# ostafen/smart

Measured on AMD Instinct MI355X. Metric: GB/s text scanned per GPU (bit-exact occ count), m=32 on 1 GiB rand128, higher is better.
Workload: dtype u8; 1 GPU; HOR m=32, 1.00 GiB rand128 per GPU; algorithm=hor, m=32, sigma=128, text_bytes_per_gpu=1073741824, patterns=2668, corpus=counter-based splitmix64 rand-sigma, seed 0x5EED0001, generated on device, ranks=1

## Files before the change

### smart_amd/csrc/api.cpp

```cpp
#include "../../include/smartgpu.h"

#include <hip/hip_runtime.h>
#include <rccl/rccl.h>

#include <dlfcn.h>

#include <algorithm>
#include <atomic>
#include <chrono>
#include <condition_variable>
#include <functional>
#include <mutex>
#include <thread>
#include <cstdarg>
#include <cstdio>
#include <cstring>
#include <string>
#include <vector>

#include "kernels.hpp"
#include "multi.hpp"
#include "multi_find.hpp"
#include "multi_find_host.hpp"
#include "pedit.hpp"
// ... 62 lines not shown
DeviceCtx* device_ctx(int device)
{
    int n = 0;
    if (hipGetDeviceCount(&n) != hipSuccess || n <= 0) {
        set_error("no HIP device available (hipGetDeviceCount)");
        return nullptr;
    }
    if (device < 0 || device >= n || device >= kMaxDevices) {
        set_error("device %d out of range (have %d)", device, n);
        return nullptr;
    }
    DeviceCtx& d = g_dev[device];
    HIP_TRY(hipSetDevice(device), return nullptr);
    if (!d.ready) {
        hipDeviceProp_t prop;
        HIP_TRY(hipGetDeviceProperties(&prop, device), return nullptr);
        d.num_cus = prop.multiProcessorCount;
        d.device = device;
        HIP_TRY(hipStreamCreateWithFlags(&d.stream, hipStreamNonBlocking), return nullptr);
        d.pinned_bytes = sg::kStagingBytes;
        HIP_TRY(hipHostMalloc(reinterpret_cast<void**>(&d.pinned), d.pinned_bytes, hipHostMallocDefault),
                return nullptr);
        HIP_TRY(hipHostMalloc(reinterpret_cast<void**>(&d.pinned_count), 64, hipHostMallocDefault),
                return nullptr);
        d.ready = true;
    }
    return &d;
}

DeviceCtx* device_ctx_ready(int device)
{
    if (device >= 0 && device < kMaxDevices && g_dev[device].ready) return &g_dev[device];
    return device_ctx(device);
}

constexpr unsigned long long kPoisonedCount = 1ull << 62;
bool count_poisoned(unsigned long long c)
{
    if (c < kPoisonedCount) return false;
    set_error("a scan kernel found its LDS segment displaced (static LDS in a kernel that addresses LDS by offset): count poisoned");
    return true;
}

double now_ms()
{
    using clk = std::chrono::steady_clock;
    return std::chrono::duration<double, std::milli>(clk::now().time_since_epoch()).count();
}

int probe_read_ms(const DeviceCtx* d, const uint8_t* first, uint64_t bytes, unsigned long long* sink, int reps, double* ms_per_pass)
{
    hipEvent_t e0 = nullptr, e1 = nullptr;
    const auto timed = [&]() -> int {
        HIP_TRY(hipEventCreate(&e0), return SMARTGPU_ERR_HIP);
        HIP_TRY(hipEventCreate(&e1), return SMARTGPU_ERR_HIP);
        sg::launch_probe_read(first, bytes, sink, d->num_cus, d->stream);
        hipEventRecord(e0, d->stream);
        for (int i = 0; i < reps; ++i) sg::launch_probe_read(first, bytes, sink, d->num_cus, d->stream);
        hipEventRecord(e1, d->stream);
        HIP_TRY(hipEventSynchronize(e1), return SMARTGPU_ERR_HIP);
        float ms = 0.f;
        hipEventElapsedTime(&ms, e0, e1);
        *ms_per_pass = ms / reps;
        return SMARTGPU_OK;
    };
    const int rc = timed();
    if (e0) hipEventDestroy(e0);
    if (e1) hipEventDestroy(e1);
    return rc;
}

}

struct smartgpu_text {
    int device = 0;
    uint64_t n = 0;
    uint8_t* base = nullptr;
    const uint8_t* data() const { return base + sg::kFrontPad; }
    uint32_t alphabet[8] = {0, 0, 0, 0, 0, 0, 0, 0};
    uint32_t four_shift = 7, four_symtab = 0, one_bit = 0xFF;
    sg::TextCodes codes() const { sg::TextCodes c; c.shift = four_shift; c.symtab = four_symtab; c.one = one_bit; return c; }
    double rate = -1.0;
    uint32_t* sample = nullptr;
};

struct smartgpu_plan {
    int device = 0;
    int algo = 0;
    uint32_t m = 0;
    sg::PlanWords words;
    uint8_t* blob = nullptr;
    uint8_t tail[sg::kTailRow] = {};
    uint8_t head[sg::kSampleRow] = {};
    unsigned long long* results = nullptr;
    unsigned long long* ext_results = nullptr;
    int ext_slots = 0;
    unsigned long long* slot_ptr(int slot) const { return ext_results ? ext_results + slot : results + slot; }
    int num_slots() const { return ext_results ? ext_slots : sg::kResultSlots; }
    hipEvent_t ev0[sg::kResultSlots] = {};
    hipEvent_t ev1[sg::kResultSlots] = {};
    bool timed[sg::kResultSlots] = {};
    double pre_ms = 0.0;
};

namespace {

smartgpu_text* text_alloc(uint64_t n, int device, DeviceCtx** ctx_out)
{
    DeviceCtx* d = device_ctx(device);
    if (!d) return nullptr;
    smartgpu_text* t = new smartgpu_text;
    t->device = device;
    t->n = n;
    const uint64_t total = sg::kFrontPad + n + sg::kBackPad;
    if (hipMalloc(reinterpret_cast<void**>(&t->base), total) != hipSuccess) {
        set_error("hipMalloc of %llu bytes failed", (unsigned long long)total);
        delete t;
        return nullptr;
    }
    if (hipMemsetAsync(t->base, 0, sg::kFrontPad, d->stream) != hipSuccess ||
        hipMemsetAsync(t->base + sg::kFrontPad + n, 0, sg::kBackPad, d->stream) != hipSuccess) {
        set_error("hipMemsetAsync of the text pads failed");
        hipFree(t->base);
        delete t;
        return nullptr;
    }
    *ctx_out = d;
    return t;
}

constexpr size_t kAlphabetScratchOff = 64;
static_assert(kAlphabetScratchOff + 32 <= sg::kFrontPad - (SMARTGPU_XSIZE + 256), "the scratch must lie below every byte a scan can read");
static_assert(sg::kHitSlotsOff >= kAlphabetScratchOff + 32 && sg::kHitSlotsOff + sg::kHitSlots * 128 <= sg::kFrontPad - (SMARTGPU_XSIZE + 256),
              "flush_hits' staging slots lie between the scratch and the bytes a scan can read");
bool text_alphabet(smartgpu_text* t, DeviceCtx* d)
{
    uint32_t* dev = reinterpret_cast<uint32_t*>(t->base + kAlphabetScratchOff);
    uint64_t hist[256] = {};
    unsigned long long* dev_hist = nullptr;
    const bool with_rate = sg::g_text_histogram && sg::rate_sample(t->n).bytes() >= 2;
    hipError_t e = hipMemsetAsync(dev, 0, 32, d->stream);
    if (e == hipSuccess && with_rate) e = hipMalloc(reinterpret_cast<void**>(&dev_hist), sizeof hist);
    if (e == hipSuccess && with_rate) e = hipMemsetAsync(dev_hist, 0, sizeof hist, d->stream);
    if (e == hipSuccess && t->n) e = sg::launch_text_alphabet(t->data(), t->n, dev, d->num_cus, d->stream);
    if (e == hipSuccess && with_rate) e = static_cast<hipError_t>(sg::g_text_histogram(t->data(), t->n, dev_hist, d->num_cus, d->stream));
    if (e == hipSuccess) e = hipMemcpyAsync(t->alphabet, dev, 32, hipMemcpyDeviceToHost, d->stream);
    if (e == hipSuccess && with_rate) e = hipMemcpyAsync(hist, dev_hist, sizeof hist, hipMemcpyDeviceToHost, d->stream);
    const hipError_t synced = hipStreamSynchronize(d->stream);
    if (e == hipSuccess) e = synced;
    if (dev_hist) (void)hipFree(dev_hist);
    if (e != hipSuccess) { set_error("text_alphabet failed: %s", hipGetErrorString(e)); return false; }
    t->rate = with_rate ? sg::text_repeat_rate(hist) : -1.0;
    if (!sg::four_symbol_codes(t->alphabet, &t->four_shift, &t->four_symtab)) t->four_shift = 7;
    t->one_bit = 0xFF;
    {
        uint32_t syms[3], ns = 0;
        for (uint32_t c = 0; c < 256 && ns < 3; ++c)
            if (t->alphabet[c >> 5] >> (c & 31) & 1u) syms[ns++] = c;
        if (ns == 1) syms[ns++] = syms[0];
        if (ns == 2) {
            uint32_t bit = 0;
            while (bit < 7 && ((syms[0] ^ syms[1]) >> bit & 1u) == 0) ++bit;
            const uint32_t s0 = (syms[0] >> bit & 1u) ? syms[1] : syms[0], s1 = (syms[0] >> bit & 1u) ? syms[0] : syms[1];
            t->one_bit = bit | (s0 << 8) | (s1 << 16);
        }
    }
    const uint32_t words[3] = {t->four_shift, t->four_symtab, t->one_bit};
    if (hipMemcpyAsync(t->base, words, 12, hipMemcpyHostToDevice, d->stream) != hipSuccess ||
        hipMemsetAsync(dev, 0, 32, d->stream) != hipSuccess ||
        hipStreamSynchronize(d->stream) != hipSuccess) {
        set_error("text_alphabet: writing the codes failed");
        return false;
    }
    return true;
}

bool text_no_alphabet(smartgpu_text* t, DeviceCtx* d)
{
    t->four_shift = 7;
    t->four_symtab = 0;
    t->one_bit = 0xFF;
    t->rate = -1.0;
    for (uint32_t& wv : t->alphabet) wv = 0xFFFFFFFFu;
    const uint32_t words[3] = {7u, 0u, 0xFFu};
    if (hipMemcpyAsync(t->base, words, 12, hipMemcpyHostToDevice, d->stream) != hipSuccess || hipStreamSynchronize(d->stream) != hipSuccess) {
        set_error("text upload: writing the codes failed");
        return false;
    }
    return true;
}

std::atomic<long long> g_text_sampling{64ll << 20};

void text_sample(smartgpu_text* t, DeviceCtx* d)
{
    const long long least = g_text_sampling.load(std::memory_order_relaxed);
    if (least < 0 || t->n < static_cast<uint64_t>(least) || !sg::g_sample_build) return;
    uint32_t* s = nullptr;
    if (hipMalloc(reinterpret_cast<void**>(&s), sg::sample_alloc_dwords(t->n) * 4) != hipSuccess) {
        (void)hipGetLastError();
        return;
    }
    if (sg::g_sample_build(t->data(), t->n, s, d->num_cus, d->stream) != hipSuccess || hipStreamSynchronize(d->stream) != hipSuccess) {
        (void)hipGetLastError();
        (void)hipFree(s);
        return;
    }
    t->sample = s;
}

int check_pattern(int algo, const uint8_t* P, uint32_t m, bool length_first = false)
{
    if (algo < 0 || algo >= SMARTGPU_NUM_ALGOS) { set_error("unknown algorithm id %d", algo); return SMARTGPU_ERR_ARG; }
    const bool na = m < sg::min_pattern(algo);
    if ((!na || length_first) && (!P || m < 1 || m > SMARTGPU_XSIZE)) { set_error("pattern length %u outside [1,%d]", m, SMARTGPU_XSIZE); return SMARTGPU_ERR_ARG; }
    if (na) { set_error("%s: not applicable for m < %u", sg::kAlgoNames[algo], sg::min_pattern(algo)); return SMARTGPU_NA; }
    return SMARTGPU_OK;
}

int check_search_args(int algo, const uint8_t* P, uint32_t m, const smartgpu_text* text,
                      uint64_t off, uint64_t n)
{
    const int rc = check_pattern(algo, P, m);
    if (rc != SMARTGPU_OK) return rc;
    if (!text) { set_error("text handle is NULL"); return SMARTGPU_ERR_ARG; }
    if (off > text->n || n > text->n - off) { set_error("range [%llu,+%llu) outside the text (%llu bytes)", (unsigned long long)off, (unsigned long long)n, (unsigned long long)text->n); return SMARTGPU_ERR_ARG; }
    return SMARTGPU_OK;
}

sg::ScanArgs make_args(const sg::PlanWords& pw, uint32_t m, const uint8_t* blob, unsigned long long* count, const smartgpu_text* text,
                       uint64_t off, uint64_t n)
{
    const uint64_t s_end = (n >= m) ? off + n - m + 1 : off;
    return sg::ScanArgs{text->data(), off, s_end, m, pw.halo,  0, pw.prefer_packed, pw.sparse, pw.so_off, blob, count};
}

struct QueuedScan { int algo; sg::ScanArgs a; sg::TextCodes codes; uint8_t tail[sg::kTailRow]; uint8_t head[sg::kSampleRow]; const uint32_t* sample; };
bool same_key(const sg::ScanArgs& x, const sg::ScanArgs& a) { return x.text == a.text && x.s_begin == a.s_begin && x.s_end == a.s_end && x.m == a.m && x.halo == a.halo; }
struct QueuedKey {
    sg::ScanArgs key;
    uint32_t n = 0;
    uint32_t streaming = 0;
    int64_t opened_ns = 0;
    bool fast = false;
    QueuedScan scans[sg::kLongMax];
    bool holds(const sg::ScanArgs& a) const { return same_key(key, a); }
    void take(const QueuedKey& o)
    {
        key = o.key;
        n = o.n;
        streaming = o.streaming;
        opened_ns = o.opened_ns;
        fast = o.fast;
        std::memcpy(static_cast<void*>(scans), static_cast<const void*>(o.scans), o.n * sizeof(QueuedScan));
    }
};
static_assert(std::is_trivially_copyable<QueuedScan>::value, "QueuedKey::take copies entries as bytes");
static_assert(SMARTGPU_XSIZE - 1 - sg::kGramCap + sg::kTailRow <= sg::kPatternBytes, "a long pass reads whole rows from a blob's pattern slot");
struct LaunchQueue {
    std::mutex mu;
    static constexpr uint32_t kKeys = 8;
    uint32_t nkeys = 0;
    QueuedKey keys[kKeys];
    void drop(uint32_t at) { for (--nkeys; at < nkeys; ++at) keys[at].take(keys[at + 1]); }
    uint32_t nfull = 0, full_next = 0;
    sg::ScanArgs full[kKeys];
    bool was_full(const sg::ScanArgs& a) const
    {
        for (uint32_t i = 0; i < nfull; ++i)
            if (same_key(full[i], a)) return true;
        return false;
    }
    void note_full(const sg::ScanArgs& a)
    {
        if (was_full(a)) return;
        if (nfull < kKeys) { full[nfull++] = a; return; }
        full[full_next] = a;
        full_next = (full_next + 1) % kKeys;
    }
    bool off = false;
    uint64_t launches = 0, passes = 0;
    uint64_t riders = 0;
    uint64_t sampled = 0;
};
LaunchQueue g_queue[kMaxDevices];
std::atomic<long long> g_coalesce_long{64ll << 20};
constexpr int kCoalesceNarrow = 8;
std::atomic<int> g_coalesce{sg::kPassMax};
std::atomic<int> g_coalesce_sample{1};
std::atomic<int> g_sample_grid{0};
bool pass_sampled(const uint32_t* sample, uint32_t m)
{
    return sample && m >= sg::kSampleMinM && sg::g_hor_sample && g_coalesce_sample.load(std::memory_order_relaxed) != 0;
}

int64_t host_ns()
{
    return std::chrono::duration_cast<std::chrono::nanoseconds>(std::chrono::steady_clock::now().time_since_epoch()).count();
}
constexpr int64_t kFastLeastNs = 10000;
int64_t pass_estimate_ns(uint64_t range, bool sampled)
{
    const uint64_t bytes = sampled ? range / (sg::kSampleStride / sg::kSampleGram) : range;
    return static_cast<int64_t>(bytes / 4400u);
}

hipError_t send_key(const DeviceCtx* d, LaunchQueue& q, QueuedKey& k)
{
    hipError_t e = k.n ? hipSetDevice(d->device) : hipSuccess;
    if (e != hipSuccess) {
        k.n = 0;
        k.streaming = 0;
        return e;
    }
    if (k.n == 1) {
        e = sg::launch_scan(k.scans[0].algo, k.scans[0].a, d->num_cus, d->stream, k.scans[0].codes);
    } else if (k.n > 1) {
        sg::MultiArgs ma;
        ma.text = k.key.text;
        ma.s_begin = k.key.s_begin;
        ma.s_end = k.key.s_end;
        ma.m = k.key.m;
        ma.halo = k.key.halo & 0xFFu;
        ma.np = k.n;
        const uint32_t* sample = k.scans[0].sample;
        if (pass_sampled(sample, k.key.m)) {
            const bool by_value = k.n <= sg::kSampleWidth;
            ma.stride = sg::kSampleRow;
            ma.width = by_value ? sg::kSampleWidth : sg::kSampleLongWidth;
            ma.reserved = by_value ? sg::kMultiByValue : sg::kMultiLong;
            for (uint32_t j = 0; j < k.n; ++j) {
                if (by_value) sg::sample_set(ma, j, k.scans[j].a.blob, k.scans[j].a.count, k.scans[j].head);
                else sg::multi_set_long(ma, j, k.scans[j].a.blob, k.scans[j].a.count);
            }
            e = sg::g_hor_sample(ma, sample, d->num_cus, g_sample_grid.load(std::memory_order_relaxed), d->stream);
            if (e == hipSuccess) ++q.sampled;
        } else {
            ma.stride = sg::tail_stride(k.key.m);
            if (k.n <= sg::pass_width(k.key.m)) {
                ma.width = sg::pass_width(k.key.m);
                ma.reserved = sg::kMultiByValue;
                for (uint32_t j = 0; j < k.n; ++j) sg::multi_set(ma, j, k.scans[j].a.blob, k.scans[j].a.count, k.scans[j].tail);
            } else {
                ma.width = sg::long_width(k.key.m);
                ma.reserved = sg::kMultiLong;
                for (uint32_t j = 0; j < k.n; ++j) sg::multi_set_long(ma, j, k.scans[j].a.blob, k.scans[j].a.count);
            }
            e = sg::g_hor_multi(ma, d->num_cus, d->stream);
        }
    }
    if (k.n && e == hipSuccess) ++q.passes;
    k.n = 0;
    k.streaming = 0;
    return e;
}

hipError_t flush_queue(const DeviceCtx* d)
{
    LaunchQueue& q = g_queue[d->device];
    std::lock_guard<std::mutex> lock(q.mu);
    hipError_t err = hipSuccess;
    for (uint32_t i = 0; i < q.nkeys; ++i) {
        const hipError_t e = send_key(d, q, q.keys[i]);
        if (e != hipSuccess && err == hipSuccess) err = e;
    }
    q.nkeys = 0;
    q.nfull = q.full_next = 0;
    return err;
}

void flush_all_queues()
{
    int current = -1;
    for (int i = 0; i < kMaxDevices; ++i) {
        if (!g_dev[i].ready) continue;
        {
            std::lock_guard<std::mutex> lock(g_queue[i].mu);
            if (g_queue[i].nkeys == 0) continue;
        }
        if (current < 0 && hipGetDevice(&current) != hipSuccess) return;
        if (hipSetDevice(i) == hipSuccess) (void)flush_queue(&g_dev[i]);
    }
    if (current >= 0) (void)hipSetDevice(current);
}

DeviceCtx* device_ctx_flushed(int device)
{
    DeviceCtx* d = device_ctx(device);
    if (!d) return nullptr;
    const hipError_t e = flush_queue(d);
    if (e != hipSuccess) { set_error("a queued launch failed: %s", hipGetErrorString(e)); return nullptr; }
    return d;
}

hipError_t queue_launch(const DeviceCtx* d, int algo, const sg::PlanWords& words, const sg::ScanArgs& a, const sg::TextCodes& codes,
                        double text_rate, const uint8_t (&tail)[sg::kTailRow], const uint8_t (&head)[sg::kSampleRow], const uint32_t* sample,
                        bool timed, bool* queued)
{
    *queued = false;
    if (a.s_end <= a.s_begin) return hipSuccess;
    const bool rider = !words.sparse;
    if (rider && (a.m < 8 || !sg::text_rate_streams(text_rate))) return hipSuccess;
    const sg::Route r = sg::route(algo, a.m, words, codes);
    if (r.to != sg::Launcher::hor || r.arg != 0) return hipSuccess;
    LaunchQueue& q = g_queue[d->device];
    std::lock_guard<std::mutex> lock(q.mu);
    if (!rider) ++q.launches;
    const int G = g_coalesce.load(std::memory_order_relaxed);
    if (timed || G < 2 || q.off || !sg::g_hor_multi) {
        if (!rider) ++q.passes;
        return hipSuccess;
    }
    hipError_t err = hipSuccess;
    uint32_t at = 0;
    while (at < q.nkeys && !q.keys[at].holds(a)) ++at;
    if (at == q.nkeys) {
        if (rider) return hipSuccess;
        if (q.nkeys == LaunchQueue::kKeys) {
            err = send_key(d, q, q.keys[0]);
            q.drop(0);
        }
        at = q.nkeys++;
        q.keys[at].key = a;
        q.keys[at].n = 0;
        q.keys[at].streaming = 0;
        q.keys[at].fast = false;
        q.keys[at].opened_ns = host_ns();
    }
    QueuedKey& k = q.keys[at];
    QueuedScan& qs = k.scans[k.n++];
    qs.algo = algo;
    qs.a = a;
    qs.codes = codes;
    std::memcpy(qs.tail, tail, sg::kTailRow);
    std::memcpy(qs.head, head, sg::kSampleRow);
    qs.sample = sample;
    if (rider) ++q.riders; else ++k.streaming;
    const bool sampled = pass_sampled(sample, a.m);
    const uint32_t room = sampled ? sg::kSampleWidth : sg::pass_width(a.m);
    const uint32_t long_room = sampled ? sg::kSampleLongWidth : sg::long_width(a.m);
    const uint32_t width = static_cast<uint32_t>(G) < room ? static_cast<uint32_t>(G) : room;
    const long long least = g_coalesce_long.load(std::memory_order_relaxed);
    const bool may_gather = G == sg::kPassMax && least >= 0 && a.s_end - a.s_begin >= static_cast<uint64_t>(least);
    const bool full = k.streaming >= width || k.n >= room;
    if (may_gather && full && !k.fast && k.n < long_room && !q.was_full(a)) {
        const int64_t waited = host_ns() - k.opened_ns;
        const int64_t pass_ns = pass_estimate_ns(a.s_end - a.s_begin, sampled);
        k.fast = pass_ns >= kFastLeastNs && waited >= 0 && waited / k.n * (long_room - k.n) < pass_ns;
    }
    const bool gather_on = may_gather && (k.fast || q.was_full(a));
    if (gather_on ? k.n >= long_room : full) {
        q.note_full(k.key);
        const hipError_t e = send_key(d, q, k);
        if (e != hipSuccess && err == hipSuccess) err = e;
        q.drop(at);
    }
    *queued = true;
    return err;
}

}

namespace sg {
hipError_t (*g_hor_multi)(const MultiArgs&, int, hipStream_t) = nullptr;
hipError_t (*g_hor_multi_find)(const MultiFindArgs&, int, hipStream_t) = nullptr;
hipError_t (*g_hor_sample)(const MultiArgs&, const uint32_t*, int, int, hipStream_t) = nullptr;
hipError_t (*g_sample_build)(const uint8_t*, uint64_t, uint32_t*, int, hipStream_t) = nullptr;
hipError_t (*g_hor_preload)() = nullptr;
int (*g_text_histogram)(const uint8_t*, uint64_t, unsigned long long*, int, void*) = nullptr;
hipError_t (*g_planes_edit_scan)(const PlaneEditArgs&, int, int, hipStream_t) = nullptr;
hipError_t (*g_planes_edit_find)(const PlaneEditArgs&, unsigned long long*, unsigned long long, int, int, hipStream_t) = nullptr;
hipError_t (*g_planes_editl_scan)(const PlaneEditlArgs&, int, int, hipStream_t) = nullptr;
hipError_t (*g_planes_editl_find)(const PlaneEditlArgs&, unsigned long long*, unsigned long long, int, int, hipStream_t) = nullptr;
hipError_t (*g_text_edit_scan)(const TextEditArgs&, int, hipStream_t) = nullptr;
hipError_t (*g_text_edit_find)(const TextEditArgs&, unsigned long long*, unsigned long long, int, hipStream_t) = nullptr;
hipError_t (*g_text_mis_scan)(const TextMisArgs&, int, hipStream_t) = nullptr;
hipError_t (*g_text_mis_find)(const TextMisArgs&, unsigned long long*, unsigned long long, int, hipStream_t) = nullptr;
hipError_t (*g_planes_edit_align)(const PlaneAlignArgs&, int, hipStream_t) = nullptr;
hipError_t (*g_text_edit_align)(const TextAlignArgs&, hipStream_t) = nullptr;
hipError_t (*g_planes3_pack)(const uint8_t*, uint64_t, uint32_t*, uint32_t*, uint32_t*, const uint8_t[7], hipStream_t) = nullptr;
hipError_t (*g_planes3_scan)(const Plane3Args&, int, int, hipStream_t) = nullptr;
hipError_t (*g_planes3_find)(const Plane3Args&, unsigned long long*, unsigned long long, int, int, hipStream_t) = nullptr;
}

extern "C" {

const char* smartgpu_version(void)
{
#ifdef SMARTGPU_AB
    return "smartgpu 0.2 (gfx950, A/B build)";
#else
    return "smartgpu 0.2 (gfx950)";
#endif
}
const char* smartgpu_last_error(void) { return g_error.c_str(); }

int smartgpu_device_count(void)
{
    int n = 0;
    if (hipGetDeviceCount(&n) != hipSuccess) { set_error("hipGetDeviceCount failed"); return SMARTGPU_ERR_HIP; }
    return n;
}

int smartgpu_algo_id(const char* name)
{
    if (!name) return -1;
    std::string s(name);
    for (auto& ch : s) ch = static_cast<char>(std::tolower(static_cast<unsigned char>(ch)));
    for (int i = 0; i < SMARTGPU_NUM_ALGOS; ++i)
        if (s == sg::kAlgoNames[i]) return i;
    return -1;
}

const char* smartgpu_algo_name(int algo)
{
    return (algo >= 0 && algo < SMARTGPU_NUM_ALGOS) ? sg::kAlgoNames[algo] : nullptr;
}

int smartgpu_device_sync(int device)
{
    DeviceCtx* d = device_ctx_flushed(device);
    if (!d) return SMARTGPU_ERR_HIP;
    HIP_TRY(hipStreamSynchronize(d->stream), return SMARTGPU_ERR_HIP);
    return SMARTGPU_OK;
}

static smartgpu_text* text_upload_impl(const void* host, uint64_t n, int device, bool alphabet)
{
    if (!host && n) { set_error("host pointer is NULL"); return nullptr; }
    DeviceCtx* d = nullptr;
    smartgpu_text* t = text_alloc(n, device, &d);
    if (!t) return nullptr;
    const uint8_t* src = static_cast<const uint8_t*>(host);
    uint8_t* dst = t->base + sg::kFrontPad;
    for (uint64_t done = 0; done < n;) {
        const size_t chunk = static_cast<size_t>(std::min<uint64_t>(d->pinned_bytes, n - done));
        std::memcpy(d->pinned, src + done, chunk);
        if (hipMemcpyAsync(dst + done, d->pinned, chunk, hipMemcpyHostToDevice, d->stream) != hipSuccess ||
            hipStreamSynchronize(d->stream) != hipSuccess) {
            set_error("text upload failed at byte %llu", (unsigned long long)done);
            smartgpu_text_free(t);
            return nullptr;
        }
        done += chunk;
    }
    hipStreamSynchronize(d->stream);
    if (!(alphabet ? text_alphabet(t, d) : text_no_alphabet(t, d))) { smartgpu_text_free(t); return nullptr; }
    if (alphabet) text_sample(t, d);
    return t;
}

smartgpu_text* smartgpu_text_upload(const void* host, uint64_t n, int device) { return text_upload_impl(host, n, device, true); }

smartgpu_text* smartgpu_text_upload_tiled(const void* unit, uint64_t unit_len, uint64_t phase,
                                          uint64_t n, int device)
{
    if (!unit || unit_len == 0) { set_error("empty unit"); return nullptr; }
    smartgpu_text* u = smartgpu_text_upload(unit, unit_len, device);
    if (!u) return nullptr;
    DeviceCtx* d = nullptr;
    smartgpu_text* t = text_alloc(n, device, &d);
    if (!t) { smartgpu_text_free(u); return nullptr; }
    hipError_t e = sg::launch_tile_fill(t->base + sg::kFrontPad, u->data(), unit_len, phase % unit_len, n, d->stream);
    if (e == hipSuccess) e = hipStreamSynchronize(d->stream);
    smartgpu_text_free(u);
    if (e != hipSuccess) {
        set_error("tile_fill failed: %s", hipGetErrorString(e));
        smartgpu_text_free(t);
        return nullptr;
    }
    if (!text_alphabet(t, d)) { smartgpu_text_free(t); return nullptr; }
    text_sample(t, d);
    return t;
}

smartgpu_text* smartgpu_text_generate(uint64_t seed, int sigma, uint64_t off, uint64_t n, int device)
{
    if (sigma < 2 || sigma > 256) { set_error("sigma %d outside [2,256]", sigma); return nullptr; }
    DeviceCtx* d = nullptr;
    smartgpu_text* t = text_alloc(n, device, &d);
    if (!t) return nullptr;
    hipError_t e = sg::launch_generate(t->base + sg::kFrontPad, seed, sigma, off, n, d->stream);
    if (e == hipSuccess) e = hipStreamSynchronize(d->stream);
    if (e != hipSuccess) {
        set_error("generate_text failed: %s", hipGetErrorString(e));
        smartgpu_text_free(t);
        return nullptr;
    }
    if (!text_alphabet(t, d)) { smartgpu_text_free(t); return nullptr; }
    text_sample(t, d);
    return t;
}

void smartgpu_text_free(smartgpu_text* t)
{
    if (!t) return;
    if (t->base) {
        hipSetDevice(t->device);
        if (t->device >= 0 && t->device < kMaxDevices && g_dev[t->device].ready) {
            const hipError_t e = flush_queue(&g_dev[t->device]);
            if (e != hipSuccess) set_error("text_free: a queued launch failed: %s", hipGetErrorString(e));
        }
        hipFree(t->base);
        if (t->sample) hipFree(t->sample);
    }
    delete t;
}
// ... 2453 lines not shown
```

### smart_amd/csrc/k_hors.hip

```cpp
#include "dev_common.hpp"
#include "launch_common.hpp"
#include "sample.hpp"

namespace sg {

__global__ __launch_bounds__(256) void text_sample_build(const uint8_t* text, uint64_t count, uint64_t alloc, uint32_t* sample)
{
    const uint64_t step = (uint64_t)gridDim.x * 256;
    for (uint64_t k = (uint64_t)blockIdx.x * 256 + threadIdx.x; k < alloc; k += step)
        sample[k] = k < count ? __builtin_nontemporal_load(reinterpret_cast<const uint32_t*>(text + k * kSampleStride)) : 0u;
}

static hipError_t launch_sample_build(const uint8_t* text, uint64_t n, uint32_t* sample, int num_cus, hipStream_t stream)
{
    const uint64_t alloc = sample_alloc_dwords(n), want = (alloc + 255) / 256;
    const uint32_t grid = (uint32_t)std::max<uint64_t>(1, std::min<uint64_t>(want, (uint64_t)num_cus * 16));
    hipLaunchKernelGGL(text_sample_build, dim3(grid), dim3(256), 0, stream, text, sample_count(n), alloc, sample);
    return hipGetLastError();
}

constexpr int kHorsInFlight = 4;
constexpr uint32_t kHorsLaneVerify = 64;
constexpr uint32_t kHorsGramsPerThread = (kSampleLongWidth * kSampleStride + kSampleThreads - 1) / kSampleThreads;

__device__ __forceinline__ const uint8_t* hors_global(unsigned long long v)
{
    typedef const __attribute__((address_space(1))) uint8_t* global_u8;
    return (const uint8_t*)reinterpret_cast<global_u8>(v);
}
__device__ __forceinline__ unsigned long long hors_area64(const MultiArgs& a, uint32_t at)
{
    return *reinterpret_cast<const unsigned long long*>(a.area + at);
}
__device__ __forceinline__ unsigned long long hors_lane(unsigned long long v, int src)
{
    const uint32_t lo = __builtin_amdgcn_readlane((uint32_t)v, src), hi = __builtin_amdgcn_readlane((uint32_t)(v >> 32), src);
    return ((unsigned long long)hi << 32) | lo;
}
__device__ __forceinline__ uint32_t hors_wave_verify(bool has, const uint8_t* tptr, const uint8_t* pptr, uint32_t len)
{
    unsigned long long todo = __ballot(has);
    const uint32_t lane = threadIdx.x & 63u;
    uint32_t mine = 0;
    while (todo) {
        const int src = __builtin_ctzll(todo);
        todo &= todo - 1;
        const uint8_t* t = hors_global(hors_lane((unsigned long long)tptr, src));
        const uint8_t* p = hors_global(hors_lane((unsigned long long)pptr, src));
        bool diff = false;
        for (uint32_t off = lane * 16u; off < len; off += 1024u)
            diff |= differ16(t + off, p + off, len - off < 16 ? len - off : 16u);
        if (!__any(diff) && lane == (uint32_t)src) mine = 1;
    }
    return mine;
}

__device__ __forceinline__ uint4 hors_quad(const uint32_t* sample, uint64_t q)
{
    return ld_stream16(reinterpret_cast<const uint8_t*>(sample + 4 * q));
}

template <int THREADS>
__global__ __launch_bounds__(THREADS) void hor_sample_scan(MultiArgs a, const uint32_t* sample)
{
    static_assert(THREADS == (int)kSampleThreads, "sample.hpp counts the LDS and the widths for this workgroup");
    constexpr int U = kHorsInFlight;
    extern __shared__ __attribute__((aligned(16))) uint8_t smem[];
    const uint32_t m = a.m, np = a.np, W = a.width;
    const bool by_value = a.reserved == kMultiByValue;
    uint32_t* filter = reinterpret_cast<uint32_t*>(smem);
    uint32_t* heads = filter + kSampleFilterWords;
    SampleEntry* entries = reinterpret_cast<SampleEntry*>(heads + kSampleBuckets);
    uint32_t* sums = reinterpret_cast<uint32_t*>(entries + np * kSampleStride);

    unsigned long long head_count = 0;
    if (threadIdx.x < np) head_count = hors_area64(a, multi_count_at(W, threadIdx.x));
    const uint32_t ngrams = np * kSampleStride;
    uint32_t mine[kHorsGramsPerThread];
#pragma unroll
    for (uint32_t r = 0; r < kHorsGramsPerThread; ++r) {
        const uint32_t idx = threadIdx.x + r * THREADS;
        mine[r] = 0;
        if (idx < ngrams) {
            const uint32_t j = idx / kSampleStride, i = idx - j * kSampleStride;
            if (by_value) mine[r] = sample_row_gram(a.area + multi_rows_at(W) + j * kSampleRow, i);
            else mine[r] = sample_row_gram(hors_global(hors_area64(a, multi_blob_at(j))), i);
        }
    }

    const uint64_t q_first = sample_quad_first(a.s_begin), q_end = sample_quad_end(a.s_end);
    const uint64_t rows = (q_end - q_first + THREADS - 1) / THREADS;
    const uint64_t per = (rows + gridDim.x - 1) / gridDim.x;
    uint64_t r = (uint64_t)blockIdx.x * per;
    const uint64_t r1 = r + per < rows ? r + per : rows;
    uint4 v[U], w[U];
    uint32_t okv = 0, okw = 0;
    auto issue = [&](uint64_t row, uint4 (&dst)[U], uint32_t& ok) {
        ok = 0;
#pragma unroll
        for (int u = 0; u < U; ++u) {
            const uint64_t q = q_first + (row + u) * THREADS + threadIdx.x;
            dst[u] = uint4{0, 0, 0, 0};
            if (row + u < r1 && q < q_end) {
                dst[u] = hors_quad(sample, q);
                ok |= 1u << u;
            }
        }
    };
    if (r < r1) issue(r, v, okv);

    {
        const uint4 zero = {0, 0, 0, 0};
        for (uint32_t j = threadIdx.x * 4u; j < kSampleFilterWords + kSampleBuckets; j += THREADS * 4u) *reinterpret_cast<uint4*>(filter + j) = zero;
        if (threadIdx.x < np) sums[threadIdx.x] = 0;
    }
    __syncthreads();
#pragma unroll
    for (uint32_t k = 0; k < kHorsGramsPerThread; ++k) {
        const uint32_t idx = threadIdx.x + k * THREADS;
        if (idx < ngrams) {
            const uint32_t j = idx / kSampleStride, i = idx - j * kSampleStride;
            const uint32_t h = sample_hash(mine[k]);
            atomicOr(filter + sample_filter_word(h), sample_filter_bit(h));
            const uint32_t next = atomicExch(heads + sample_bucket(h), idx + 1u);
            entries[idx] = SampleEntry{mine[k], sample_link(j, i, next)};
        }
    }
    __syncthreads();

    const bool wave_wide = m > kHorsLaneVerify;
    for (; r < r1; r += U) {
        if (r + U < r1) issue(r + U, w, okw); else okw = 0;
        uint32_t mask = 0;
#pragma unroll
        for (int u = 0; u < U; ++u) {
            const uint32_t g[4] = {v[u].x, v[u].y, v[u].z, v[u].w};
#pragma unroll
            for (int c = 0; c < 4; ++c) {
                const uint32_t h = sample_hash(g[c]);
                mask |= ((filter[sample_filter_word(h)] >> (h & 31u)) & 1u) << (4 * u + c);
            }
        }
#pragma unroll
        for (int u = 0; u < U; ++u)
            if (!(okv >> u & 1u)) mask &= ~(0xFu << (4 * u));
        const uint64_t k0 = 4u * (q_first + r * THREADS + threadIdx.x);
        bool parked = false;
        uint32_t parked_j = 0;
        const uint8_t* parked_at = a.text;
        unsigned long long parked_blob = (unsigned long long)a.text;
        while (mask) {
            const uint32_t b = (uint32_t)__builtin_ctz(mask);
            mask &= mask - 1u;
            uint32_t gram = 0;
#pragma unroll
            for (int u = 0; u < U; ++u) {
                gram = b == 4u * u ? v[u].x : gram;
                gram = b == 4u * u + 1u ? v[u].y : gram;
                gram = b == 4u * u + 2u ? v[u].z : gram;
                gram = b == 4u * u + 3u ? v[u].w : gram;
            }
            const uint64_t p = (k0 + (uint64_t)(b >> 2) * (4u * THREADS) + (b & 3u)) * kSampleStride;
            for (uint32_t e = heads[sample_bucket(sample_hash(gram))]; e != 0;) {
                const SampleEntry ent = entries[e - 1u];
                e = sample_link_next(ent.link);
                uint64_t s;
                if (ent.gram != gram || !sample_window(p, sample_link_offset(ent.link), a.s_begin, a.s_end, &s)) continue;
                const uint32_t j = sample_link_pattern(ent.link);
                const unsigned long long blob = hors_area64(a, multi_blob_at(j));
                const uint8_t* at = a.text + s;
                if (wave_wide && !parked) {
                    parked = true;
                    parked_at = at;
                    parked_j = j;
                    parked_blob = blob;
                } else if (global_equal(at, hors_global(blob), m)) {
                    atomicAdd(sums + j, 1u);
                }
            }
        }
        if (wave_wide && hors_wave_verify(parked, parked_at, hors_global(parked_blob), m)) atomicAdd(sums + parked_j, 1u);
#pragma unroll
        for (int u = 0; u < U; ++u) v[u] = w[u];
        okv = okw;
    }

    __syncthreads();
    if (threadIdx.x < np && sums[threadIdx.x] != 0) {
        typedef __attribute__((address_space(1))) unsigned long long* global_u64;
        atomicAdd((unsigned long long*)reinterpret_cast<global_u64>(head_count), (unsigned long long)sums[threadIdx.x]);
    }
}

static hipError_t launch_hor_sample(const MultiArgs& a, const uint32_t* sample, int num_cus, int grid_want, hipStream_t stream)
{
    if (!sample || a.m < kSampleMinM || (a.reserved != kMultiByValue && a.reserved != kMultiLong)) return hipErrorInvalidValue;
    const bool by_value = a.reserved == kMultiByValue;
    if (a.width != (by_value ? kSampleWidth : kSampleLongWidth) || a.stride != kSampleRow || a.np < 1 || a.np > a.width) return hipErrorInvalidValue;
    if (a.s_end <= a.s_begin) return hipSuccess;
    const uint64_t rows = (sample_quad_end(a.s_end) - sample_quad_first(a.s_begin) + kSampleThreads - 1) / kSampleThreads;
    uint64_t grid = grid_want > 0 ? (uint64_t)grid_want : (uint64_t)num_cus;
    if (grid > rows) grid = rows;
    const uint64_t least = (rows + (1u << 15) - 1) >> 15;
    if (grid < least) grid = least;
    const size_t lds = sample_lds(a.np);
    const void* kernel = reinterpret_cast<const void*>(&hor_sample_scan<(int)kSampleThreads>);
    allow_lds(kernel, sample_lds(kSampleLongWidth));
    hipLaunchKernelGGL((hor_sample_scan<(int)kSampleThreads>), dim3((uint32_t)grid), dim3(kSampleThreads), lds, stream, a, sample);
    return hipGetLastError();
}

namespace {
struct RegisterHorSample {
    RegisterHorSample()
    {
        g_hor_sample = &launch_hor_sample;
        g_sample_build = &launch_sample_build;
    }
} g_register_hor_sample;
}

}
```

### smart_amd/csrc/sample.hpp

```cpp
#pragma once
#include "multi.hpp"

namespace sg {

constexpr uint32_t kSampleStride = 28;
constexpr uint32_t kSampleGram = 4;
constexpr uint32_t kSampleMinM = kSampleStride + kSampleGram - 1;
static_assert(kSampleStride % 4 == 0 && kSampleGram == 4, "every sampled gram is an aligned dword of the text");

__host__ __device__ constexpr uint64_t sample_count(uint64_t n) { return (n + 2 * kSampleStride - 1) / kSampleStride; }
__host__ __device__ constexpr uint64_t sample_alloc_dwords(uint64_t n) { return ((sample_count(n) + 3) & ~3ull) + 4; }
static_assert(sample_count(0) == 1 && sample_count(1) == 2 && sample_count(28) == 2 && sample_count(29) == 3, "k runs over 28k < n + 28");

constexpr uint32_t kSampleRow = 32;
__host__ __device__ inline void sample_head_fill(uint8_t* row, const uint8_t* P, uint32_t m)
{
    for (uint32_t j = 0; j < kSampleRow; ++j) row[j] = j < m && j < kSampleMinM ? P[j] : (uint8_t)0;
}
__host__ __device__ inline uint32_t sample_row_gram(const uint8_t* row, uint32_t i)
{
    uint32_t g;
    __builtin_memcpy(&g, row + i, 4);
    return g;
}

constexpr uint32_t kSampleFilterBits = 19;
constexpr uint32_t kSampleFilterWords = 1u << (kSampleFilterBits - 5);
__host__ __device__ inline uint32_t sample_hash(uint32_t gram) { return (gram * 0x9E3779B1u) >> (32 - kSampleFilterBits); }
__host__ __device__ inline uint32_t sample_filter_word(uint32_t h) { return h >> 5; }
__host__ __device__ inline uint32_t sample_filter_bit(uint32_t h) { return 1u << (h & 31u); }
constexpr uint32_t kSampleBuckets = 4096;
__host__ __device__ inline uint32_t sample_bucket(uint32_t h) { return h >> (kSampleFilterBits - 12); }
struct SampleEntry { uint32_t gram, link; };
__host__ __device__ inline uint32_t sample_link(uint32_t j, uint32_t i, uint32_t next) { return j | (i << 8) | (next << 16); }
__host__ __device__ inline uint32_t sample_link_pattern(uint32_t link) { return link & 0xFFu; }
__host__ __device__ inline uint32_t sample_link_offset(uint32_t link) { return (link >> 8) & 0x1Fu; }
__host__ __device__ inline uint32_t sample_link_next(uint32_t link) { return link >> 16; }

__host__ __device__ inline bool sample_window(uint64_t p, uint32_t i, uint64_t s_begin, uint64_t s_end, uint64_t* s)
{
    if (p < i) return false;
    *s = p - i;
    return *s >= s_begin && *s < s_end;
}
__host__ __device__ inline uint64_t sample_quad_first(uint64_t s_begin) { return (s_begin + kSampleStride - 1) / kSampleStride / 4; }
__host__ __device__ inline uint64_t sample_quad_end(uint64_t s_end) { return (s_end + kSampleStride - 2) / kSampleStride / 4 + 1; }

constexpr uint32_t kSampleThreads = 1024;
constexpr uint32_t kSampleLdsMax = 160u * 1024u;
__host__ __device__ constexpr uint32_t sample_lds(uint32_t np) { return 4u * kSampleFilterWords + 4u * kSampleBuckets + np * kSampleStride * 8u + 4u * np; }
constexpr uint32_t kSampleWidth = kMultiArea / (16u + kSampleRow);
constexpr uint32_t kSampleLongWidth = kMultiArea / 16u;
static_assert(kSampleWidth == 84 && kSampleLongWidth == 252 && kSampleLongWidth <= kLongMax, "a key gathers at most kLongMax entries");
static_assert(kSampleLongWidth <= 256 && kSampleLongWidth * kSampleStride < 65536, "a pattern fits the link's 8 bits, an entry index its 16");
static_assert(sample_lds(kSampleLongWidth) <= kSampleLdsMax && kSampleLongWidth <= kSampleThreads, "the widest pass fits one CU's LDS, a thread per pattern");
static_assert(kSampleMinM <= kSampleRow && kSampleRow % 16 == 0, "a row holds every gram a pass enters");

inline void sample_set(MultiArgs& a, uint32_t g, const uint8_t* blob, unsigned long long* count, const uint8_t* row)
{
    __builtin_memcpy(a.area + multi_blob_at(g), &blob, 8);
    __builtin_memcpy(a.area + multi_count_at(a.width, g), &count, 8);
    __builtin_memcpy(a.area + multi_rows_at(a.width) + g * kSampleRow, row, kSampleRow);
}

extern hipError_t (*g_hor_sample)(const MultiArgs& a, const uint32_t* sample, int num_cus, int grid, hipStream_t stream);
extern hipError_t (*g_sample_build)(const uint8_t* text, uint64_t n, uint32_t* sample, int num_cus, hipStream_t stream);

}
```

Measured before the change: 377,000 GB/s.

## Add two-bit filter, staged prefetch ring, and fast-path loads in sampled HOR scan

Each sample gram now sets two bits in the same filter word, and a probe tests both with one word load plus a rotate. The aim is to cut the false-positive rate that drives bucket-chain walks. The prefetch is restructured into a STAGES-deep ring with an unguarded fast path when a full group of quads is in bounds, which removes the per-quad bounds checks and the register copy of the next group. Gram selection after a hit becomes a select tree instead of a linear scan. The host pass-time estimate constant is also adjusted. The extra bit raises filter density, which could offset part of the gain.

```diff
diff --git a/smart_amd/csrc/api.cpp b/smart_amd/csrc/api.cpp
--- a/smart_amd/csrc/api.cpp
+++ b/smart_amd/csrc/api.cpp
@@ -388,7 +388,7 @@
 int64_t pass_estimate_ns(uint64_t range, bool sampled)
 {
     const uint64_t bytes = sampled ? range / (sg::kSampleStride / sg::kSampleGram) : range;
-    return static_cast<int64_t>(bytes / 4400u);
+    return static_cast<int64_t>(bytes / 4600u);
 }
 
 hipError_t send_key(const DeviceCtx* d, LaunchQueue& q, QueuedKey& k)
diff --git a/smart_amd/csrc/k_hors.hip b/smart_amd/csrc/k_hors.hip
--- a/smart_amd/csrc/k_hors.hip
+++ b/smart_amd/csrc/k_hors.hip
@@ -20,6 +20,7 @@
 }
 
 constexpr int kHorsInFlight = 4;
+constexpr int kHorsStages = 2;
 constexpr uint32_t kHorsLaneVerify = 64;
 constexpr uint32_t kHorsGramsPerThread = (kSampleLongWidth * kSampleStride + kSampleThreads - 1) / kSampleThreads;
 
@@ -64,7 +65,7 @@
 __global__ __launch_bounds__(THREADS) void hor_sample_scan(MultiArgs a, const uint32_t* sample)
 {
     static_assert(THREADS == (int)kSampleThreads, "sample.hpp counts the LDS and the widths for this workgroup");
-    constexpr int U = kHorsInFlight;
+    constexpr int U = kHorsInFlight, STAGES = kHorsStages;
     extern __shared__ __attribute__((aligned(16))) uint8_t smem[];
     const uint32_t m = a.m, np = a.np, W = a.width;
     const bool by_value = a.reserved == kMultiByValue;
@@ -93,21 +94,30 @@
     const uint64_t per = (rows + gridDim.x - 1) / gridDim.x;
     uint64_t r = (uint64_t)blockIdx.x * per;
     const uint64_t r1 = r + per < rows ? r + per : rows;
-    uint4 v[U], w[U];
-    uint32_t okv = 0, okw = 0;
-    auto issue = [&](uint64_t row, uint4 (&dst)[U], uint32_t& ok) {
-        ok = 0;
+    uint4 v[STAGES][U];
+    uint32_t ok[STAGES];
+    constexpr uint32_t kAll = (1u << U) - 1u;
+    auto issue = [&](uint64_t row, uint4 (&dst)[U], uint32_t& have) {
+        if (row + U <= r1 && q_first + (row + U) * THREADS <= q_end) {
+            const uint64_t q = q_first + row * THREADS + threadIdx.x;
+#pragma unroll
+            for (int u = 0; u < U; ++u) dst[u] = hors_quad(sample, q + (uint64_t)u * THREADS);
+            have = kAll;
+            return;
+        }
+        have = 0;
 #pragma unroll
         for (int u = 0; u < U; ++u) {
             const uint64_t q = q_first + (row + u) * THREADS + threadIdx.x;
             dst[u] = uint4{0, 0, 0, 0};
             if (row + u < r1 && q < q_end) {
                 dst[u] = hors_quad(sample, q);
-                ok |= 1u << u;
+                have |= 1u << u;
             }
         }
     };
-    if (r < r1) issue(r, v, okv);
+#pragma unroll
+    for (int s = 0; s < STAGES - 1; ++s) issue(r + (uint64_t)s * U, v[s], ok[s]);
 
     {
         const uint4 zero = {0, 0, 0, 0};
@@ -120,8 +130,8 @@
         const uint32_t idx = threadIdx.x + k * THREADS;
         if (idx < ngrams) {
             const uint32_t j = idx / kSampleStride, i = idx - j * kSampleStride;
-            const uint32_t h = sample_hash(mine[k]);
-            atomicOr(filter + sample_filter_word(h), sample_filter_bit(h));
+            const uint32_t product = sample_product(mine[k]), h = sample_product_hash(product);
+            atomicOr(filter + sample_filter_word(h), sample_filter_pair(product));
             const uint32_t next = atomicExch(heads + sample_bucket(h), idx + 1u);
             entries[idx] = SampleEntry{mine[k], sample_link(j, i, next)};
         }
@@ -129,22 +139,25 @@
     __syncthreads();
 
     const bool wave_wide = m > kHorsLaneVerify;
-    for (; r < r1; r += U) {
-        if (r + U < r1) issue(r + U, w, okw); else okw = 0;
+    auto step = [&](uint64_t row, const uint4 (&cur)[U], uint32_t have) {
         uint32_t mask = 0;
 #pragma unroll
         for (int u = 0; u < U; ++u) {
-            const uint32_t g[4] = {v[u].x, v[u].y, v[u].z, v[u].w};
+            const uint32_t g[4] = {cur[u].x, cur[u].y, cur[u].z, cur[u].w};
 #pragma unroll
             for (int c = 0; c < 4; ++c) {
-                const uint32_t h = sample_hash(g[c]);
-                mask |= ((filter[sample_filter_word(h)] >> (h & 31u)) & 1u) << (4 * u + c);
-            }
-        }
-#pragma unroll
-        for (int u = 0; u < U; ++u)
-            if (!(okv >> u & 1u)) mask &= ~(0xFu << (4 * u));
-        const uint64_t k0 = 4u * (q_first + r * THREADS + threadIdx.x);
+                const uint32_t product = sample_product(g[c]);
+                const uint32_t word = filter[sample_filter_word(sample_product_hash(product))];
+                const uint32_t both = word & __builtin_amdgcn_alignbit(word, word, sample_filter_distance(product));
+                mask = (__builtin_amdgcn_ubfe(both, sample_product_hash(product), 1u) << (4 * u + c)) | mask;
+            }
+        }
+        if (have != kAll) {
+#pragma unroll
+            for (int u = 0; u < U; ++u)
+                if (!(have >> u & 1u)) mask &= ~(0xFu << (4 * u));
+        }
+        const uint64_t k0 = 4u * (q_first + row * THREADS + threadIdx.x);
         bool parked = false;
         uint32_t parked_j = 0;
         const uint8_t* parked_at = a.text;
@@ -152,14 +165,9 @@
         while (mask) {
             const uint32_t b = (uint32_t)__builtin_ctz(mask);
             mask &= mask - 1u;
-            uint32_t gram = 0;
-#pragma unroll
-            for (int u = 0; u < U; ++u) {
-                gram = b == 4u * u ? v[u].x : gram;
-                gram = b == 4u * u + 1u ? v[u].y : gram;
-                gram = b == 4u * u + 2u ? v[u].z : gram;
-                gram = b == 4u * u + 3u ? v[u].w : gram;
-            }
+            static_assert(U == 4, "the tree below");
+            const uint4 lo = b & 4u ? cur[1] : cur[0], hi = b & 4u ? cur[3] : cur[2], quad = b & 8u ? hi : lo;
+            const uint32_t gram = b & 2u ? (b & 1u ? quad.w : quad.z) : (b & 1u ? quad.y : quad.x);
             const uint64_t p = (k0 + (uint64_t)(b >> 2) * (4u * THREADS) + (b & 3u)) * kSampleStride;
             for (uint32_t e = heads[sample_bucket(sample_hash(gram))]; e != 0;) {
                 const SampleEntry ent = entries[e - 1u];
@@ -180,9 +188,17 @@
             }
         }
         if (wave_wide && hors_wave_verify(parked, parked_at, hors_global(parked_blob), m)) atomicAdd(sums + parked_j, 1u);
-#pragma unroll
-        for (int u = 0; u < U; ++u) v[u] = w[u];
-        okv = okw;
+    };
+    while (r < r1) {
+#pragma unroll
+        for (int s = 0; s < STAGES; ++s) {
+            if (r < r1) {
+                constexpr int kLast = STAGES - 1;
+                issue(r + (uint64_t)kLast * U, v[(s + kLast) % STAGES], ok[(s + kLast) % STAGES]);
+                step(r, v[s], ok[s]);
+                r += U;
+            }
+        }
     }
 
     __syncthreads();
diff --git a/smart_amd/csrc/sample.hpp b/smart_amd/csrc/sample.hpp
--- a/smart_amd/csrc/sample.hpp
+++ b/smart_amd/csrc/sample.hpp
@@ -29,6 +29,19 @@
 __host__ __device__ inline uint32_t sample_hash(uint32_t gram) { return (gram * 0x9E3779B1u) >> (32 - kSampleFilterBits); }
 __host__ __device__ inline uint32_t sample_filter_word(uint32_t h) { return h >> 5; }
 __host__ __device__ inline uint32_t sample_filter_bit(uint32_t h) { return 1u << (h & 31u); }
+constexpr uint32_t kSampleProductShift = 32 - kSampleFilterBits;
+__host__ __device__ inline uint32_t sample_product(uint32_t gram) { return gram * 0x9E3779B1u; }
+__host__ __device__ inline uint32_t sample_product_hash(uint32_t product) { return product >> kSampleProductShift; }
+__host__ __device__ inline uint32_t sample_filter_distance(uint32_t product) { return (product & 31u) | 1u; }
+__host__ __device__ inline uint32_t sample_filter_index2(uint32_t product)
+{
+    return (sample_product_hash(product) + sample_filter_distance(product)) & 31u;
+}
+__host__ __device__ inline uint32_t sample_filter_bit2(uint32_t gram) { return 1u << sample_filter_index2(sample_product(gram)); }
+__host__ __device__ inline uint32_t sample_filter_pair(uint32_t product)
+{
+    return sample_filter_bit(sample_product_hash(product)) | (1u << sample_filter_index2(product));
+}
 constexpr uint32_t kSampleBuckets = 4096;
 __host__ __device__ inline uint32_t sample_bucket(uint32_t h) { return h >> (kSampleFilterBits - 12); }
 struct SampleEntry { uint32_t gram, link; };
```

Result: slower. 342,400 GB/s (-9.2%).

## Rotate sample prefetch buffers and hash filter probes with direct LDS addressing

Applied to the files above, without the earlier changes.

Restructures the sampled HOR scan loop into a rotating multi-buffer prefetch (depth configurable) with 32-bit offsets from a per-block base, replacing the double-buffer copy and per-row bounds masks. The filter and bucket lookups now hash once with a multiplicative constant and compute LDS byte addresses directly (assuming the filter sits at LDS offset zero), and a bitfield extract replaces the shift-and-mask. Gram selection on a hit uses a two-level select instead of a 16-way chain. The aim is to cut scalar/ALU overhead and address arithmetic in the memory-bound loop. It adds a runtime check that refuses launch if static LDS is nonzero, and it inlines the hash, which must match sample_hash for correctness.

```diff
diff --git a/smart_amd/csrc/k_hors.hip b/smart_amd/csrc/k_hors.hip
--- a/smart_amd/csrc/k_hors.hip
+++ b/smart_amd/csrc/k_hors.hip
@@ -19,7 +19,15 @@
     return hipGetLastError();
 }
 
-constexpr int kHorsInFlight = 4;
+#ifndef SMARTGPU_HORS_INFLIGHT
+#define SMARTGPU_HORS_INFLIGHT 4
+#endif
+#ifndef SMARTGPU_HORS_DEPTH
+#define SMARTGPU_HORS_DEPTH 1
+#endif
+constexpr int kHorsInFlight = SMARTGPU_HORS_INFLIGHT;
+constexpr int kHorsDepth = SMARTGPU_HORS_DEPTH;
+static_assert(kHorsInFlight >= 1 && kHorsInFlight <= 4 && kHorsDepth >= 1, "a step's mask has 16 bits; the rotation needs a batch ahead");
 constexpr uint32_t kHorsLaneVerify = 64;
 constexpr uint32_t kHorsGramsPerThread = (kSampleLongWidth * kSampleStride + kSampleThreads - 1) / kSampleThreads;
 
@@ -55,16 +63,31 @@
     return mine;
 }
 
-__device__ __forceinline__ uint4 hors_quad(const uint32_t* sample, uint64_t q)
-{
-    return ld_stream16(reinterpret_cast<const uint8_t*>(sample + 4 * q));
+constexpr uint32_t kHorsHashMul = 0x9E3779B1u;
+__device__ __forceinline__ uint32_t hors_filter_word(uint32_t x)
+{
+    typedef const __attribute__((address_space(3))) uint32_t* lds_u32;
+    return *(lds_u32)(uintptr_t)((x >> (32 - kSampleFilterBits + 5 - 2)) & (4u * (kSampleFilterWords - 1u)));
+}
+__device__ __forceinline__ uint32_t hors_chain_head(uint32_t x)
+{
+    typedef const __attribute__((address_space(3))) uint32_t* lds_u32;
+    static_assert((4u * kSampleFilterWords & (4u * kSampleFilterWords - 1u)) == 0 && kSampleBuckets <= kSampleFilterWords, "the offset is OR-ed in");
+    static_assert(kSampleBuckets == 1u << 12, "sample_bucket takes the hash's top 12 bits");
+    return *(lds_u32)(uintptr_t)(((x >> (32 - 12 - 2)) & (4u * (kSampleBuckets - 1u))) | (4u * kSampleFilterWords));
+}
+
+typedef uint32_t hors_u32x4 __attribute__((ext_vector_type(4)));
+__device__ __forceinline__ hors_u32x4 hors_quad(const uint8_t* first, uint32_t at)
+{
+    return __builtin_nontemporal_load(reinterpret_cast<const hors_u32x4*>(first + at));
 }
 
 template <int THREADS>
 __global__ __launch_bounds__(THREADS) void hor_sample_scan(MultiArgs a, const uint32_t* sample)
 {
     static_assert(THREADS == (int)kSampleThreads, "sample.hpp counts the LDS and the widths for this workgroup");
-    constexpr int U = kHorsInFlight;
+    constexpr int U = kHorsInFlight, D = kHorsDepth + 1;
     extern __shared__ __attribute__((aligned(16))) uint8_t smem[];
     const uint32_t m = a.m, np = a.np, W = a.width;
     const bool by_value = a.reserved == kMultiByValue;
@@ -91,23 +114,19 @@
     const uint64_t q_first = sample_quad_first(a.s_begin), q_end = sample_quad_end(a.s_end);
     const uint64_t rows = (q_end - q_first + THREADS - 1) / THREADS;
     const uint64_t per = (rows + gridDim.x - 1) / gridDim.x;
-    uint64_t r = (uint64_t)blockIdx.x * per;
-    const uint64_t r1 = r + per < rows ? r + per : rows;
-    uint4 v[U], w[U];
-    uint32_t okv = 0, okw = 0;
-    auto issue = [&](uint64_t row, uint4 (&dst)[U], uint32_t& ok) {
-        ok = 0;
-#pragma unroll
-        for (int u = 0; u < U; ++u) {
-            const uint64_t q = q_first + (row + u) * THREADS + threadIdx.x;
-            dst[u] = uint4{0, 0, 0, 0};
-            if (row + u < r1 && q < q_end) {
-                dst[u] = hors_quad(sample, q);
-                ok |= 1u << u;
-            }
-        }
+    const uint64_t r0 = (uint64_t)blockIdx.x * per;
+    const uint32_t cnt = r0 < rows ? (uint32_t)(r0 + per < rows ? per : rows - r0) : 0u;
+    const uint64_t q0 = cnt ? q_first + r0 * THREADS : 0;
+    const uint32_t own = cnt && q0 + (uint64_t)(cnt - 1u) * THREADS + threadIdx.x >= q_end ? cnt - 1u : cnt;
+    const uint8_t* const base = reinterpret_cast<const uint8_t*>(sample + 4 * q0);
+    const uint32_t lane_at = threadIdx.x * 16u;
+    auto issue = [&](uint32_t row, hors_u32x4 (&dst)[U]) {
+#pragma unroll
+        for (int u = 0; u < U; ++u) dst[u] = hors_quad(base, row + u < own ? lane_at + (row + u) * (THREADS * 16u) : 0u);
     };
-    if (r < r1) issue(r, v, okv);
+    hors_u32x4 v[D][U];
+#pragma unroll
+    for (int k = 0; k + 1 < D; ++k) issue(k * U, v[k]);
 
     {
         const uint4 zero = {0, 0, 0, 0};
@@ -129,22 +148,27 @@
     __syncthreads();
 
     const bool wave_wide = m > kHorsLaneVerify;
-    for (; r < r1; r += U) {
-        if (r + U < r1) issue(r + U, w, okw); else okw = 0;
+    const uint64_t p0 = 4u * q0 * kSampleStride;
+    auto step = [&](uint32_t row, const hors_u32x4 (&v)[U]) {
         uint32_t mask = 0;
 #pragma unroll
-        for (int u = 0; u < U; ++u) {
-            const uint32_t g[4] = {v[u].x, v[u].y, v[u].z, v[u].w};
-#pragma unroll
-            for (int c = 0; c < 4; ++c) {
-                const uint32_t h = sample_hash(g[c]);
-                mask |= ((filter[sample_filter_word(h)] >> (h & 31u)) & 1u) << (4 * u + c);
+        for (int u0 = 0; u0 < U; u0 += 2) {
+            constexpr int kPair = 8;
+            uint32_t h[kPair], word[kPair];
+#pragma unroll
+            for (int t = 0; t < kPair; ++t) {
+                const hors_u32x4 q = v[u0 + t / 4 < U ? u0 + t / 4 : u0];
+                const uint32_t x = (t % 4 == 0 ? q.x : t % 4 == 1 ? q.y : t % 4 == 2 ? q.z : q.w) * kHorsHashMul;
+                h[t] = x >> (32 - kSampleFilterBits);
+                word[t] = hors_filter_word(x);
             }
-        }
-#pragma unroll
-        for (int u = 0; u < U; ++u)
-            if (!(okv >> u & 1u)) mask &= ~(0xFu << (4 * u));
-        const uint64_t k0 = 4u * (q_first + r * THREADS + threadIdx.x);
+#pragma unroll
+            for (int t = 0; t < kPair; ++t)
+                if (u0 + t / 4 < U) mask |= __builtin_amdgcn_ubfe(word[t], h[t], 1u) << (4 * u0 + t);
+        }
+        const uint32_t have = own - row < (uint32_t)U ? own - row : (uint32_t)U;
+        mask &= (1u << (4u * have)) - 1u;
+        const uint32_t at0 = row * (4u * THREADS * kSampleStride) + threadIdx.x * (4u * kSampleStride);
         bool parked = false;
         uint32_t parked_j = 0;
         const uint8_t* parked_at = a.text;
@@ -152,16 +176,19 @@
         while (mask) {
             const uint32_t b = (uint32_t)__builtin_ctz(mask);
             mask &= mask - 1u;
-            uint32_t gram = 0;
-#pragma unroll
-            for (int u = 0; u < U; ++u) {
-                gram = b == 4u * u ? v[u].x : gram;
-                gram = b == 4u * u + 1u ? v[u].y : gram;
-                gram = b == 4u * u + 2u ? v[u].z : gram;
-                gram = b == 4u * u + 3u ? v[u].w : gram;
+            const uint32_t bu = b >> 2, bc = b & 3u;
+            hors_u32x4 q = v[0];
+#pragma unroll
+            for (int u = 1; u < U; ++u) {
+                q.x = bu == (uint32_t)u ? v[u].x : q.x;
+                q.y = bu == (uint32_t)u ? v[u].y : q.y;
+                q.z = bu == (uint32_t)u ? v[u].z : q.z;
+                q.w = bu == (uint32_t)u ? v[u].w : q.w;
             }
-            const uint64_t p = (k0 + (uint64_t)(b >> 2) * (4u * THREADS) + (b & 3u)) * kSampleStride;
-            for (uint32_t e = heads[sample_bucket(sample_hash(gram))]; e != 0;) {
+            const uint32_t lo = bc & 1u ? q.y : q.x, hi = bc & 1u ? q.w : q.z;
+            const uint32_t gram = bc & 2u ? hi : lo;
+            const uint64_t p = p0 + (at0 + bu * (4u * THREADS * kSampleStride) + bc * kSampleStride);
+            for (uint32_t e = hors_chain_head(gram * kHorsHashMul); e != 0;) {
                 const SampleEntry ent = entries[e - 1u];
                 e = sample_link_next(ent.link);
                 uint64_t s;
@@ -180,9 +207,14 @@
             }
         }
         if (wave_wide && hors_wave_verify(parked, parked_at, hors_global(parked_blob), m)) atomicAdd(sums + parked_j, 1u);
-#pragma unroll
-        for (int u = 0; u < U; ++u) v[u] = w[u];
-        okv = okw;
+    };
+    for (uint32_t row = 0; row < cnt;) {
+#pragma unroll
+        for (int k = 0; k < D; ++k) {
+            issue(row + (D - 1) * U, v[(k + D - 1) % D]);
+            if (row < cnt) step(row, v[k]);
+            row += U;
+        }
     }
 
     __syncthreads();
@@ -205,6 +237,11 @@
     if (grid < least) grid = least;
     const size_t lds = sample_lds(a.np);
     const void* kernel = reinterpret_cast<const void*>(&hor_sample_scan<(int)kSampleThreads>);
+    static const bool filter_at_zero = [kernel] {
+        hipFuncAttributes at{};
+        return hipFuncGetAttributes(&at, kernel) == hipSuccess && at.sharedSizeBytes == 0;
+    }();
+    if (!filter_at_zero) return hipErrorInvalidValue;
     allow_lds(kernel, sample_lds(kSampleLongWidth));
     hipLaunchKernelGGL((hor_sample_scan<(int)kSampleThreads>), dim3((uint32_t)grid), dim3(kSampleThreads), lds, stream, a, sample);
     return hipGetLastError();
```

Result: slower. 393,300 GB/s before, 367,100 GB/s after (-6.7%).
